# VincentStimper/normalizing-flows

Measured on NVIDIA H100. Metric: samples/sec forward_kld, 32-layer RQ-NSF d=64 batch=65536, higher is better.
Workload: dtype f32

## Files before the change

### normalizing-flows_b200/csrc/nfb_common.cuh

```cuda
#pragma once
#include <cuda_runtime.h>
#include <cuda_bf16.h>
#include <cuda_fp16.h>
#include <stdint.h>
#include <stdio.h>

#define NFB_OK 0
#define NFB_ERR_CUDA 1
#define NFB_ERR_ARG 2
#define NFB_ERR_UNSUPPORTED 3
#define NFB_ERR_STATE 4

void nfb_set_error(const char* fmt, ...);

#define NFB_CUDA(call)                                                                   \
    do {                                                                                 \
        cudaError_t e__ = (call);                                                        \
        if (e__ != cudaSuccess) {                                                        \
            nfb_set_error("%s:%d: %s -> %s", __FILE__, __LINE__, #call,                  \
                          cudaGetErrorString(e__));                                      \
            return NFB_ERR_CUDA;                                                         \
        }                                                                                \
    } while (0)

// ... 7 lines not shown

#define NFB_LAUNCH_CHECK() NFB_CUDA(cudaGetLastError())

namespace nfb {

constexpr float kMinBinWidth = 1e-3f;
constexpr float kMinBinHeight = 1e-3f;
constexpr float kMinDerivative = 1e-3f;
constexpr float kLog2e = 1.4426950408889634f;
constexpr float kLn2 = 0.6931471805599453f;

__device__ __forceinline__ uint32_t smem_u32(const void* p) {
    return static_cast<uint32_t>(__cvta_generic_to_shared(p));
}

__device__ __forceinline__ bool elect_one_sync() {
    uint32_t pred = 0;
    asm volatile(
        "{\n\t.reg .b32 %%rx;\n\t.reg .pred %%px;\n\t"
        "elect.sync %%rx|%%px, %1;\n\t"
        "@%%px mov.s32 %0, 1;\n\t}"
        : "+r"(pred)
        : "r"(0xffffffffu));
    return pred != 0;
}

__device__ __forceinline__ void mbar_init(uint32_t bar, uint32_t count) {
    asm volatile("mbarrier.init.shared::cta.b64 [%0], %1;" ::"r"(bar), "r"(count) : "memory");
}
__device__ __forceinline__ void fence_mbar_init() {
    asm volatile("fence.mbarrier_init.release.cluster;" ::: "memory");
}
__device__ __forceinline__ void mbar_arrive(uint32_t bar) {
    asm volatile("mbarrier.arrive.shared::cta.b64 _, [%0];" ::"r"(bar) : "memory");
}
__device__ __forceinline__ void mbar_expect_tx(uint32_t bar, uint32_t bytes) {
    asm volatile("mbarrier.arrive.expect_tx.shared::cta.b64 _, [%0], %1;" ::"r"(bar), "r"(bytes)
                 : "memory");
}
__device__ __forceinline__ bool mbar_try_wait(uint32_t bar, uint32_t parity) {
    uint32_t ok;
    asm volatile(
        "{\n\t.reg .pred p;\n\t"
        "mbarrier.try_wait.parity.shared::cta.b64 p, [%1], %2;\n\t"
        "selp.u32 %0, 1, 0, p;\n\t}"
        : "=r"(ok)
        : "r"(bar), "r"(parity)
        : "memory");
    return ok != 0;
}
static __device__ __noinline__ void fail_timeout(int* err, int tag) {
    if (err) atomicExch(err, tag);
    __threadfence_system();
    asm volatile("trap;");
}

__device__ __forceinline__ void mbar_wait(uint32_t bar, uint32_t parity, int* err, int tag) {
    if (mbar_try_wait(bar, parity)) return;
    long long t0 = clock64();
    while (!mbar_try_wait(bar, parity)) {
        if (clock64() - t0 > 4000000000LL) fail_timeout(err, tag);
    }
}

__device__ __forceinline__ void mbar_wait_warp(uint32_t bar, uint32_t parity, int* err, int tag) {
    if ((threadIdx.x & 31) == 0 && !mbar_try_wait(bar, parity)) {
        long long t0 = clock64();
        while (!mbar_try_wait(bar, parity)) {
            if (clock64() - t0 > 4000000000LL) fail_timeout(err, tag);
        }
    }
    __syncwarp();
}

__device__ __forceinline__ void bulk_g2s(uint32_t dst_smem, const void* src, uint32_t bytes,
                                         uint32_t bar) {
    asm volatile(
        "cp.async.bulk.shared::cluster.global.mbarrier::complete_tx::bytes [%0], [%1], %2, [%3];"
        ::"r"(dst_smem), "l"(src), "r"(bytes), "r"(bar)
        : "memory");
}
__device__ __forceinline__ void fence_proxy_async_smem() {
    asm volatile("fence.proxy.async.shared::cta;" ::: "memory");
}

__device__ __forceinline__ uint64_t wgmma_desc(uint32_t smem_addr, uint32_t lbo16 = 1, uint32_t sbo16 = 64) {
    return (uint64_t)((smem_addr & 0x3FFFFu) >> 4) | ((uint64_t)lbo16 << 16) | ((uint64_t)sbo16 << 32) | (1ull << 62);
}
__device__ __forceinline__ void wgmma_fence() { asm volatile("wgmma.fence.sync.aligned;" ::: "memory"); }
__device__ __forceinline__ void wgmma_commit() { asm volatile("wgmma.commit_group.sync.aligned;" ::: "memory"); }
template <int N> __device__ __forceinline__ void wgmma_wait() {
    asm volatile("wgmma.wait_group.sync.aligned %0;" ::"n"(N) : "memory");
}
template <int R> __device__ __forceinline__ void wgmma_hold(float (&d)[R]) {
#pragma unroll
    for (int i = 0; i < R; ++i) asm volatile("" : "+f"(d[i])::"memory");
}
__device__ __forceinline__ void wgmma_f16_n64(float (&d)[32], uint64_t a, uint64_t b, uint32_t scale_d) {
    asm volatile(
        "{\n\t.reg .pred p;\n\tsetp.ne.b32 p, %34, 0;\n\t"
        "wgmma.mma_async.sync.aligned.m64n64k16.f32.f16.f16 "
        "{"
        "%0,%1,%2,%3,%4,%5,%6,%7,%8,%9,%10,%11,%12,%13,%14,%15,"
        "%16,%17,%18,%19,%20,%21,%22,%23,%24,%25,%26,%27,%28,%29,%30,%31"
        "}, %32, %33, p, 1, 1, 0, 0;\n\t}"
        : "+f"(d[0]), "+f"(d[1]), "+f"(d[2]), "+f"(d[3]), "+f"(d[4]), "+f"(d[5]), "+f"(d[6]), "+f"(d[7]), "+f"(d[8]),
          "+f"(d[9]), "+f"(d[10]), "+f"(d[11]), "+f"(d[12]), "+f"(d[13]), "+f"(d[14]), "+f"(d[15]), "+f"(d[16]),
          "+f"(d[17]), "+f"(d[18]), "+f"(d[19]), "+f"(d[20]), "+f"(d[21]), "+f"(d[22]), "+f"(d[23]), "+f"(d[24]),
          "+f"(d[25]), "+f"(d[26]), "+f"(d[27]), "+f"(d[28]), "+f"(d[29]), "+f"(d[30]), "+f"(d[31])
        : "l"(a), "l"(b), "r"(scale_d));
}
__device__ __forceinline__ void wgmma_f16_n96(float (&d)[48], uint64_t a, uint64_t b, uint32_t scale_d) {
    asm volatile(
        "{\n\t.reg .pred p;\n\tsetp.ne.b32 p, %50, 0;\n\t"
        "wgmma.mma_async.sync.aligned.m64n96k16.f32.f16.f16 "
        "{"
        "%0,%1,%2,%3,%4,%5,%6,%7,%8,%9,%10,%11,%12,%13,%14,%15,"
        "%16,%17,%18,%19,%20,%21,%22,%23,%24,%25,%26,%27,%28,%29,%30,%31,"
        "%32,%33,%34,%35,%36,%37,%38,%39,%40,%41,%42,%43,%44,%45,%46,%47"
        "}, %48, %49, p, 1, 1, 0, 0;\n\t}"
        : "+f"(d[0]), "+f"(d[1]), "+f"(d[2]), "+f"(d[3]), "+f"(d[4]), "+f"(d[5]), "+f"(d[6]), "+f"(d[7]), "+f"(d[8]),
          "+f"(d[9]), "+f"(d[10]), "+f"(d[11]), "+f"(d[12]), "+f"(d[13]), "+f"(d[14]), "+f"(d[15]), "+f"(d[16]),
          "+f"(d[17]), "+f"(d[18]), "+f"(d[19]), "+f"(d[20]), "+f"(d[21]), "+f"(d[22]), "+f"(d[23]), "+f"(d[24]),
          "+f"(d[25]), "+f"(d[26]), "+f"(d[27]), "+f"(d[28]), "+f"(d[29]), "+f"(d[30]), "+f"(d[31]), "+f"(d[32]),
          "+f"(d[33]), "+f"(d[34]), "+f"(d[35]), "+f"(d[36]), "+f"(d[37]), "+f"(d[38]), "+f"(d[39]), "+f"(d[40]),
          "+f"(d[41]), "+f"(d[42]), "+f"(d[43]), "+f"(d[44]), "+f"(d[45]), "+f"(d[46]), "+f"(d[47])
        : "l"(a), "l"(b), "r"(scale_d));
}
__device__ __forceinline__ void wgmma_f16_n64_zero(float (&d)[32], uint64_t a, uint64_t b) {
    asm volatile(
        "wgmma.mma_async.sync.aligned.m64n64k16.f32.f16.f16 "
        "{"
        "%0,%1,%2,%3,%4,%5,%6,%7,%8,%9,%10,%11,%12,%13,%14,%15,"
        "%16,%17,%18,%19,%20,%21,%22,%23,%24,%25,%26,%27,%28,%29,%30,%31"
        "}, %32, %33, 0, 1, 1, 0, 0;"
        : "=f"(d[0]), "=f"(d[1]), "=f"(d[2]), "=f"(d[3]), "=f"(d[4]), "=f"(d[5]), "=f"(d[6]), "=f"(d[7]), "=f"(d[8]),
          "=f"(d[9]), "=f"(d[10]), "=f"(d[11]), "=f"(d[12]), "=f"(d[13]), "=f"(d[14]), "=f"(d[15]), "=f"(d[16]),
          "=f"(d[17]), "=f"(d[18]), "=f"(d[19]), "=f"(d[20]), "=f"(d[21]), "=f"(d[22]), "=f"(d[23]), "=f"(d[24]),
          "=f"(d[25]), "=f"(d[26]), "=f"(d[27]), "=f"(d[28]), "=f"(d[29]), "=f"(d[30]), "=f"(d[31])
        : "l"(a), "l"(b));
}
__device__ __forceinline__ void wgmma_f16_n96_zero(float (&d)[48], uint64_t a, uint64_t b) {
    asm volatile(
        "wgmma.mma_async.sync.aligned.m64n96k16.f32.f16.f16 "
        "{"
        "%0,%1,%2,%3,%4,%5,%6,%7,%8,%9,%10,%11,%12,%13,%14,%15,"
        "%16,%17,%18,%19,%20,%21,%22,%23,%24,%25,%26,%27,%28,%29,%30,%31,"
        "%32,%33,%34,%35,%36,%37,%38,%39,%40,%41,%42,%43,%44,%45,%46,%47"
        "}, %48, %49, 0, 1, 1, 0, 0;"
        : "=f"(d[0]), "=f"(d[1]), "=f"(d[2]), "=f"(d[3]), "=f"(d[4]), "=f"(d[5]), "=f"(d[6]), "=f"(d[7]), "=f"(d[8]),
          "=f"(d[9]), "=f"(d[10]), "=f"(d[11]), "=f"(d[12]), "=f"(d[13]), "=f"(d[14]), "=f"(d[15]), "=f"(d[16]),
          "=f"(d[17]), "=f"(d[18]), "=f"(d[19]), "=f"(d[20]), "=f"(d[21]), "=f"(d[22]), "=f"(d[23]), "=f"(d[24]),
          "=f"(d[25]), "=f"(d[26]), "=f"(d[27]), "=f"(d[28]), "=f"(d[29]), "=f"(d[30]), "=f"(d[31]), "=f"(d[32]),
          "=f"(d[33]), "=f"(d[34]), "=f"(d[35]), "=f"(d[36]), "=f"(d[37]), "=f"(d[38]), "=f"(d[39]), "=f"(d[40]),
          "=f"(d[41]), "=f"(d[42]), "=f"(d[43]), "=f"(d[44]), "=f"(d[45]), "=f"(d[46]), "=f"(d[47])
        : "l"(a), "l"(b));
}
template <int TA = 0, int TB = 0>
__device__ __forceinline__ void wgmma_bf16_n64(float (&d)[32], uint64_t a, uint64_t b, uint32_t scale_d, uint32_t on = 1) {
    asm volatile(
        "{\n\t.reg .pred p, q;\n\tsetp.ne.b32 p, %34, 0;\n\tsetp.ne.b32 q, %37, 0;\n\t"
        "@q wgmma.mma_async.sync.aligned.m64n64k16.f32.bf16.bf16 "
        "{"
        "%0,%1,%2,%3,%4,%5,%6,%7,%8,%9,%10,%11,%12,%13,%14,%15,"
        "%16,%17,%18,%19,%20,%21,%22,%23,%24,%25,%26,%27,%28,%29,%30,%31"
        "}, %32, %33, p, 1, 1, %35, %36;\n\t}"
// ... 61 lines not shown
```

### normalizing-flows_b200/csrc/nfb_fused_rqs.cu

```cuda
#include <type_traits>

#include "nfb_kernels.h"
#include "nfb_spline.cuh"

namespace nfb {

constexpr int kRows = kFusedTileRows;
constexpr int kCons = 256;
constexpr int kFusedThreads = kCons + 128;
constexpr int kProducerRegs = 24, kConsumerRegs = 240;
constexpr uint32_t kTileA = 8192;
constexpr uint32_t kSlotBytes = 32768;
constexpr uint32_t kSlots = 3;
constexpr uint32_t kOffW = 8 * kTileA;
constexpr uint32_t kOffX = kOffW + kSlots * kSlotBytes;
constexpr int kStgLd = 52;
constexpr uint32_t kStgBytes = kRows * kStgLd * 4;
constexpr uint32_t kOffStg = kOffX + kRows * 64 * 4;
constexpr uint32_t kOffMisc = kOffStg + 2 * kStgBytes;
constexpr uint32_t kOffBars = kOffMisc + 4 * kRows * 4;
constexpr uint32_t kNumBars = 10;
constexpr uint32_t kOffUnitQ = kOffBars + kNumBars * 8;
constexpr uint32_t kFusedSmem = kOffUnitQ + 32;
static_assert(kFusedSmem <= 232448, "shared memory budget");
static_assert(2 * kFusedFeaturesPerChunk * 24 * 64 * 4 <= (int)kSlotBytes, "final-layer record must fit a ring slot");

constexpr int kBarWFull = 0 , kBarWEmpty = 3 , kBarUnit = 6 ;

__device__ __forceinline__ uint32_t xs_index(int r, int c) { return r * 64 + (c ^ (r & 31)); }

__device__ __forceinline__ uint32_t a_chunk_off(int r, int c8) {
    return (r >> 3) * 1024 + (r & 7) * 128 + ((c8 ^ (r & 7)) << 4);
}

__device__ __forceinline__ void st_shared_v4(uint32_t addr, uint32_t a, uint32_t b, uint32_t c,
                                             uint32_t d) {
    asm volatile("st.shared.v4.b32 [%0], {%1,%2,%3,%4};" ::"r"(addr), "r"(a), "r"(b), "r"(c), "r"(d)
                 : "memory");
}
__device__ __forceinline__ void cons_bar_sync() {
    asm volatile("bar.sync 1, %0;" ::"n"(kCons) : "memory");
}
constexpr int kBarStgFull = 2, kBarStgFree = 3;
template <int ID> __device__ __forceinline__ void stg_bar_arrive() {
    __threadfence_block();
    asm volatile("bar.arrive %0, %1;" ::"n"(ID), "n"(kCons) : "memory");
}
template <int ID> __device__ __forceinline__ void stg_bar_wait() {
    asm volatile("bar.sync %0, %1;" ::"n"(ID), "n"(kCons) : "memory");
}
__device__ __forceinline__ void mbar_arrive_if(uint32_t bar, bool pred) {
    asm volatile("{\n\t.reg .pred p;\n\tsetp.ne.b32 p, %1, 0;\n\t@p mbarrier.arrive.shared::cta.b64 _, [%0];\n\t}"
                 ::"r"(bar), "r"((uint32_t)pred) : "memory");
}

__device__ __forceinline__ void split_store8(const float* v, uint32_t t0, uint32_t t1, uint32_t off) {
    uint32_t h[4], l[4];
#pragma unroll
    for (int i = 0; i < 4; ++i) {
        const float a = v[2 * i], b = v[2 * i + 1];
        h[i] = pack_f16x2(a, b);
        const float2 hf = unpack_f16x2(h[i]);
        l[i] = pack_f16x2(a - hf.x, b - hf.y);
    }
    st_shared_v4(t0 + off, h[0], h[1], h[2], h[3]);
    st_shared_v4(t1 + off, l[0], l[1], l[2], l[3]);
}
template <typename T> __device__ __forceinline__ T uniform(T v) {
    return (T)__shfl_sync(0xffffffffu, (int)v, 0);
}
__device__ __forceinline__ float pow2i(int e) { return __uint_as_float((uint32_t)(127 + e) << 23); }

struct MmaOps { uint32_t a_hi, a_lo, w_hi, w_lo, on, slabs; };
template <int SLABS, bool QUAD, int NREG, bool FIRST = false>
__device__ __forceinline__ void mma_record(float (&acc)[NREG], const MmaOps& x) {
    static_assert(NREG == 32 || NREG == 48, "N = 64 or 96");
    const uint64_t ah = wgmma_desc(x.a_hi), al = wgmma_desc(x.a_lo), bh = wgmma_desc(x.w_hi), bl = wgmma_desc(x.w_lo);
    auto pass = [&](uint64_t a, uint64_t b, bool opens) {
#pragma unroll
        for (int s = 0; s < SLABS; ++s) {
            if constexpr (NREG == 32) {
                if (FIRST && opens && s == 0) wgmma_f16_n64_zero(acc, a, b);
                else wgmma_f16_n64(acc, a + 2 * s, b + 2 * s, 1u);
            } else {
                if (FIRST && opens && s == 0) wgmma_f16_n96_zero(acc, a, b);
                else wgmma_f16_n96(acc, a + 2 * s, b + 2 * s, 1u);
            }
        }
    };
    pass(ah, bh, true);
    pass(al, bh, false);
    pass(ah, bl, false);
    if constexpr (QUAD) pass(al, bl, false);
}

enum { kClkClaim,
       kClkLoad,
       kClkLu,
       kClkHidRing,
       kClkHidMma,
       kClkHidEpi,
       kClkFinRing,
       kClkFinMma,
       kClkFinTail,
       kClkFinStage,
       kClkFinSpline,
       kClkStore,
       kClkProdEmpty,
       kClkProdOther,
       kClkUnits,
       kClkCount };
template <int RING, int MMA, int TAIL> struct WalkClk { static constexpr int ring = RING, mma = MMA, tail = TAIL; };
using LuClk = WalkClk<kClkLu, kClkLu, kClkLu>;
using HidClk = WalkClk<kClkHidRing, kClkHidMma, kClkHidMma>;
using FinClk = WalkClk<kClkFinRing, kClkFinMma, kClkFinTail>;
#ifdef NFB_PHASE_CLOCKS
__device__ unsigned long long g_phase_clocks[3][kClkCount];
struct PhaseClock {
    uint32_t last, sum[kClkCount];
    __device__ PhaseClock() {
        last = (uint32_t)clock64();
#pragma unroll
        for (int i = 0; i < kClkCount; ++i) sum[i] = 0;
    }
    template <int P> __device__ __forceinline__ void stamp() {
        const uint32_t t = (uint32_t)clock64();
        sum[P] += t - last;
        last = t;
    }
    __device__ void flush(int role) const {
#pragma unroll
        for (int i = 0; i < kClkCount; ++i) atomicAdd(&g_phase_clocks[role][i], (unsigned long long)sum[i]);
    }
};
#define NFB_CLK_BEGIN() PhaseClock clk
#define NFB_CLK(P) clk.template stamp<P>()
#define NFB_CLK_UNIT() (++clk.sum[kClkUnits])
#define NFB_CLK_END(role, pred) do { if (pred) clk.flush(role); } while (0)
#else
#define NFB_CLK_BEGIN() ((void)0)
#define NFB_CLK(P) ((void)0)
#define NFB_CLK_UNIT() ((void)0)
#define NFB_CLK_END(role, pred) ((void)0)
#endif

template <bool SAMPLE>
__global__ void __launch_bounds__(kFusedThreads, 1) fused_rqs_kernel(const FusedParams p) {
    extern __shared__ __align__(1024) uint8_t smem[];
    const uint32_t sbase = smem_u32(smem);
    const int warp = uniform((int)(threadIdx.x >> 5)), lane = threadIdx.x & 31;
    float* xs = reinterpret_cast<float*>(smem + kOffX);
    float* ldsum = reinterpret_cast<float*>(smem + kOffMisc);
    int* rowexp = reinterpret_cast<int*>(smem + kOffMisc + 3 * kRows * 4);
    float* rowmax = reinterpret_cast<float*>(smem + kOffStg);
    const uint32_t bars = sbase + kOffBars;
    auto bar = [bars](int i) { return bars + 8u * i; };

    if ((sbase & 1023u) != 0) {
        if (threadIdx.x == 0 && p.err) atomicExch(p.err, 900);
        return;
    }
    if (threadIdx.x == 0) {
        for (int i = 0; i < (int)kSlots; ++i) {
            mbar_init(bar(kBarWFull + i), 1);
            mbar_init(bar(kBarWEmpty + i), 2);
        }
        for (int i = 0; i < 4; ++i) mbar_init(bar(kBarUnit + i), 1);
        fence_mbar_init();
    }
    __syncthreads();

    volatile int* unit_q = reinterpret_cast<volatile int*>(smem + kOffUnitQ);
    if (warp >= kCons / 32) {
        setmaxnreg_dec<kProducerRegs>();
        if (warp != kCons / 32) return;
        const long long n_tiles = (p.rows + kRows - 1) / kRows;
        const long long n_units = n_tiles * p.n_layers;
        auto decode = [&](long long u, int& cursor, int& layer, long long& tile) {
            if (!p.wave_order) {
                layer = (int)(u / n_tiles);
                tile = u - (long long)layer * n_tiles;
                return;
            }
            while (cursor + 1 < p.wave_elems && u >= (long long)__ldg(p.wave_order + 2 * (cursor + 1) + 1)) ++cursor;
            const uint32_t w = __ldg(p.wave_order + 2 * cursor);
            layer = (int)(w & 0xffu);
            tile = (long long)(w >> 8) * p.wave_tpg + (u - (long long)__ldg(p.wave_order + 2 * cursor + 1));
        };
        uint32_t slot = 0, par = 0;
        int wcur = 0;
        NFB_CLK_BEGIN();
        for (uint32_t ui = 0;; ++ui) {
            long long u;
            if (p.ticket) {
                int t = 0;
                if (lane == 0) t = atomicAdd(p.ticket, 1);
                u = (long long)__shfl_sync(0xffffffffu, t, 0);
            } else {
                u = (long long)blockIdx.x + (long long)ui * gridDim.x;
            }
            const bool more = u < n_units;
            int ulayer = -1;
            long long utile = 0;
            if (more) decode(u, wcur, ulayer, utile);
            if (lane == 0) {
                unit_q[2 * (ui & 3u)] = ulayer;
                unit_q[2 * (ui & 3u) + 1] = (int)utile;
                mbar_arrive(bar(kBarUnit + (ui & 3u)));
            }
            __syncwarp();
            if (!more) break;
            NFB_CLK_UNIT();
            const FusedLayer& L = p.layers[ulayer];
            const FusedStep* steps = L.steps;
            const int n_steps = L.n_steps;
            const int lu_steps = L.has_lu ? 1 : 0;
            const int reps = (SAMPLE && L.ar_passes > 0) ? L.ar_passes : 1;
            const int total = n_steps ? lu_steps + reps * (n_steps - lu_steps) : 0;
            const uint32_t lu_bytes = L.has_lu ? 2u * 8192u : 0u;
            int s = 0;
            uint32_t off = 0;
            uint32_t bytes = total ? (uint32_t)__ldg(&steps[0].bytes16) << 4 : 0u;
            for (int i = 0; i < total; ++i) {
                int sn = s + 1;
                uint32_t offn = off + bytes;
                if (sn == n_steps) { sn = lu_steps; offn = lu_bytes; }
                const uint32_t nbytes = i + 1 < total ? (uint32_t)__ldg(&steps[sn].bytes16) << 4 : 0u;
                NFB_CLK(kClkProdOther);
                mbar_wait(bar(kBarWEmpty + slot), par ^ 1, p.err, 100 + slot);
                NFB_CLK(kClkProdEmpty);
                if (elect_one_sync()) {
                    mbar_expect_tx(bar(kBarWFull + slot), bytes);
                    bulk_g2s(sbase + kOffW + slot * kSlotBytes, L.wstream + off, bytes, bar(kBarWFull + slot));
                }
                __syncwarp();
                s = sn;
                off = offn;
                bytes = nbytes;
                if (++slot == kSlots) { slot = 0; par ^= 1; }
            }
        }
        NFB_CLK(kClkProdOther);
        NFB_CLK_END(2, lane == 0);
        return;
    }

    setmaxnreg_inc<kConsumerRegs>();
    const int et = threadIdx.x;
    const int wg = uniform(et >> 7);
    const int wl = warp & 3;
    const int ra = 16 * wl + (lane >> 2);
    const int rb = ra + 8;
    const int cq = 2 * (lane & 3);
    const uint32_t aA = sbase;
    float* stg0 = reinterpret_cast<float*>(smem + kOffStg);
    uint32_t slot = 0, wpar = 0;
    NFB_CLK_BEGIN();

    for (uint32_t ui = 0;; ++ui) {
        mbar_wait(bar(kBarUnit + (ui & 3u)), (ui >> 2) & 1u, p.err, 600 + (int)(ui & 3u));
        const int layer = uniform(unit_q[2 * (ui & 3u)]);
        const long long tile = uniform(unit_q[2 * (ui & 3u) + 1]);
        if (layer < 0) break;
        NFB_CLK_UNIT();
        const FusedLayer& L = p.layers[layer];
        const int D = L.D;
        auto own = [&](int q) { return uniform((int)L.own[wg][q]); };
        const int n_steps = uniform(L.n_steps), lu_steps = uniform(L.has_lu ? 1 : 0);
        const int n_hidden = uniform(L.n_hidden), n_pairs = uniform(L.n_chunks >> 1);
        int sidx = 0;
        auto hand_back = [&](auto arrivals, int s, bool pred) {
#pragma unroll
            for (int i = 0; i < decltype(arrivals)::value; ++i) mbar_arrive_if(bar(kBarWEmpty + s), pred && (et & 127) == 0);
        };
        auto walk_records = [&](auto issue, auto arrivals, auto phases, int& prev, auto open, auto retire) {
            using Clk = decltype(phases);
            auto record = [&](auto first) {
                union { uint2 raw; FusedStep s; } st;
                st.raw = __ldg(reinterpret_cast<const uint2*>(L.steps) + sidx);
                st.raw.x = uniform(st.raw.x);
                st.raw.y = uniform(st.raw.y);
                sidx = sidx + 1 == n_steps ? lu_steps : sidx + 1;
                NFB_CLK(Clk::mma);
                mbar_wait(bar(kBarWFull + slot), wpar, p.err, 220 + slot);
                NFB_CLK(Clk::ring);
                wgmma_fence();
                const bool last = issue(st.s, first);
                if constexpr (decltype(first)::value) NFB_CLK(Clk::mma);
                wgmma_wait<1>();
                hand_back(arrivals, prev < 0 ? 0 : prev, prev >= 0);
                if constexpr (decltype(first)::value) NFB_CLK(Clk::tail);
                prev = (int)slot;
                if (++slot == kSlots) { slot = 0; wpar ^= 1; }
                return last;
            };
            bool last = false;
            if constexpr (decltype(open)::value) {
                last = record(std::true_type());
                retire();
            }
            while (!last) last = record(std::false_type());
        };
        auto half_ops = [&](const FusedStep& s, int h) {
            const uint32_t kc = h ? s.kc1 : s.kc, fl = h ? s.flags1 : s.flags;
            const uint32_t w = sbase + kOffW + slot * kSlotBytes + ((fl & kStepHalf) ? 0u : (uint32_t)h * s.n8 * 1024u);
            return MmaOps{aA + kc * kTileA, aA + (4 + kc) * kTileA, w, w + ((uint32_t)s.bytes16 << 3),
                          (uint32_t)!(fl & kStepSkip), 4u - ((fl >> kStepSlabShift) & 3u)};
        };
        auto slice_products = [&](float (&acc)[32], auto opens, auto quad) {
            return [&](const FusedStep& s, auto first) {
                constexpr bool Q = decltype(quad)::value;
                const MmaOps x = half_ops(s, wg);
                if constexpr (decltype(first)::value && decltype(opens)::value) {
                    mma_record<4, Q, 32, true>(acc, x);
                    wgmma_commit();
                } else if (x.on) {
                    mma_record<4, Q, 32>(acc, x);
                    wgmma_commit();
                } else {
                    wgmma_commit();
                }
                return ((wg ? s.flags1 : s.flags) & kStepLast) != 0;
            };
        };
        auto no_products = [&](const FusedStep& s, auto) {
            wgmma_commit();
            return ((wg ? s.flags1 : s.flags) & kStepLast) != 0;
        };
        using One = std::integral_constant<int, 1>;
        using NoQuad = std::integral_constant<bool, false>;

        float* zdst = p.zout + (long long)layer * p.z_stride;
        const float* zsrc = layer == 0 ? p.zin : p.zout + (long long)(layer - 1) * p.z_stride;
        const long long row0 = tile * kRows;
        const int r = et & (kRows - 1);
        const int rq = et >> 6;
        const long long grow = row0 + r;
        const bool row_live = grow < p.rows;

        if (layer > 0) {
            if (lane == 0) {
                const int* flag = p.progress + tile;
                int seen;
                const long long t0 = clock64();
                do {
                    asm volatile("ld.acquire.gpu.global.s32 %0, [%1];" : "=r"(seen) : "l"(flag) : "memory");
                    if (seen < layer && clock64() - t0 > 4000000000LL) fail_timeout(p.err, 500);
                } while (seen < layer);
            }
            __syncwarp();
            {
                int seen;
                asm volatile("ld.acquire.gpu.global.s32 %0, [%1];" : "=r"(seen) : "l"(p.progress + tile) : "memory");
                if (seen < layer) fail_timeout(p.err, 501);
            }
        }
        if (layer == 0 && p.in_ready) {
            const int need = (int)min(row0 + kRows, p.rows);
            if (lane == 0) {
                int seen;
                const long long t0 = clock64();
                do {
                    asm volatile("ld.acquire.sys.global.s32 %0, [%1];" : "=r"(seen) : "l"(p.in_ready) : "memory");
                    if (seen < need && clock64() - t0 > 20000000000LL) fail_timeout(p.err, 510);
                } while (seen < need);
            }
            __syncwarp();
            {
                int seen;
                asm volatile("ld.acquire.sys.global.s32 %0, [%1];" : "=r"(seen) : "l"(p.in_ready) : "memory");
                if (seen < need) fail_timeout(p.err, 511);
            }
        }
        NFB_CLK(kClkClaim);
        float lq_old = 0.f;
        if (rq == 2 && row_live && (layer > 0 || p.accumulate)) lq_old = __ldcg(p.logq + grow);
        if (D == 64) {
            float4 v[kRows * 16 / kCons];
#pragma unroll
            for (int k = 0; k < kRows * 16 / kCons; ++k) {
                const int i4 = et + k * kCons, rr = i4 >> 4;
                const long long gr = row0 + rr;
                v[k] = gr < p.rows ? __ldcg(reinterpret_cast<const float4*>(zsrc + gr * 64) + (i4 & 15))
                                   : make_float4(0.f, 0.f, 0.f, 0.f);
            }
#pragma unroll
            for (int k = 0; k < kRows * 16 / kCons; ++k) {
                const int i4 = et + k * kCons, rr = i4 >> 4, c0 = (i4 & 15) * 4;
                xs[xs_index(rr, c0)] = v[k].x;
                xs[xs_index(rr, c0 + 1)] = v[k].y;
                xs[xs_index(rr, c0 + 2)] = v[k].z;
                xs[xs_index(rr, c0 + 3)] = v[k].w;
                float m = fmaxf(fmaxf(fabsf(v[k].x), fabsf(v[k].y)), fmaxf(fabsf(v[k].z), fabsf(v[k].w)));
                m = fmaxf(m, __shfl_xor_sync(0xffffffffu, m, 1));
                m = fmaxf(m, __shfl_xor_sync(0xffffffffu, m, 2));
                m = fmaxf(m, __shfl_xor_sync(0xffffffffu, m, 4));
                m = fmaxf(m, __shfl_xor_sync(0xffffffffu, m, 8));
                if ((et & 15) == 0) rowmax[rr] = m;
            }
        } else {
            for (int i = et; i < kRows * D; i += kCons) {
                const int rr = i / D, cc = i - rr * D;
                const long long gr = row0 + rr;
                xs[xs_index(rr, cc)] = gr < p.rows ? __ldcg(zsrc + gr * D + cc) : 0.f;
            }
        }
        cons_bar_sync();
        auto set_row_exp = [&](float zmax) {
            int e = (int)((__float_as_uint(zmax) >> 23) & 0xffu) - 126;
            rowexp[r] = max(0, min(126, e));
        };
        if (rq == 0) {
            float zmax = 0.f;
            if (D == 64) zmax = rowmax[r];
            else
                for (int c = 0; c < D; ++c) zmax = fmaxf(zmax, fabsf(xs[xs_index(r, c)]));
            set_row_exp(zmax);
        }
        cons_bar_sync();
        auto ru = [&](float s, int row) { return s * pow2i(-rowexp[row]); };
        auto ruinv = [&](float s, int row) { return s * pow2i(rowexp[row]); };
        auto get_x = [&](int c) -> float { return xs[xs_index(r, c)]; };
        auto put_y = [&](int c, float y) { xs[xs_index(r, c)] = y; };
        const int ar = et >> 2, aq = et & 3;
        auto store_a = [&](auto value, float sc_base) {
            const float sc = ru(sc_base, ar);
            float v[16];
#pragma unroll
            for (int j = 0; j < 16; ++j) v[j] = value(aq * 16 + j) * sc;
#pragma unroll
            for (int g = 0; g < 2; ++g) split_store8(v + 8 * g, aA, aA + 4 * kTileA, a_chunk_off(ar, 2 * aq + g));
            fence_proxy_async_smem();
            cons_bar_sync();
        };
        auto build_a_net = [&]() {
            store_a([&](int k) {
                const int c = L.in_idx[k];
                return c >= 0 ? xs[xs_index(ar, c)] : 0.f;
            }, L.a_sc[1]);
        };
        float ladsum = 0.f, lad_even = 0.f;
        const bool folded = uniform(!SAMPLE && L.has_lu && L.fold_lu);
        if (lu_steps) {
            store_a([&](int k) { return k < D ? xs[xs_index(ar, k)] : 0.f; }, L.a_sc[0]);
            NFB_CLK(kClkLoad);
            int prev = -1;
            if (wg == 0) {
                float acc[32];
                walk_records(slice_products(acc, std::true_type(), std::true_type()), One(), LuClk(), prev,
                             std::true_type(), [] {});
                wgmma_wait<0>();
                hand_back(One(), prev, true);
                wgmma_hold(acc);
                const float ia = ruinv(L.a_inv[0], ra), ib = ruinv(L.a_inv[0], rb);
#pragma unroll
                for (int i = 0; i < 32; ++i) {
                    const int c = 8 * (i >> 2) + cq + (i & 1);
                    const int rr = (i & 2) ? rb : ra;
                    if (c < D) xs[xs_index(rr, c)] = fmaf(acc[i], (i & 2) ? ib : ia, __ldg(L.bias_lu + c));
                }
            } else {
                walk_records(no_products, One(), LuClk(), prev, std::false_type(), [] {});
                wgmma_wait<0>();
                hand_back(One(), prev, true);
            }
            cons_bar_sync();
            NFB_CLK(kClkLu);
        }
// ... 169 lines not shown
                int prev = -1;
                auto pair = [&](float (&acc)[48], float (&done)[48], int ci) __attribute__((always_inline)) {
                    walk_records(products(acc), Two(), FinClk(), prev, std::true_type(), [&] { stage(done, ci - 1); });
                };
                auto finish = [&](float (&acc)[48], int ci) {
                    wgmma_wait<0>();
                    hand_back(Two(), prev, true);
                    NFB_CLK(kClkFinTail);
                    stage(acc, ci);
                };
                float accA[48], accB[48];
                if (n_pairs > 0) {
                    load_bias(0);
                    walk_records(products(accA), Two(), FinClk(), prev, std::true_type(), [] {});
                    for (int ci = 1;; ci += 2) {
                        if (ci == n_pairs) { finish(accA, ci - 1); break; }
                        pair(accB, accA, ci);
                        if (ci + 1 == n_pairs) { finish(accB, ci); break; }
                        pair(accA, accB, ci + 1);
                    }
                }
            } else {
                if (n_pairs > 0) {
                    const uint32_t adv = slot + (uint32_t)(n_steps - sidx);
                    slot = adv % kSlots;
                    wpar ^= (adv / kSlots) & 1u;
                    sidx = lu_steps;
                }
                const int f = (et >> 6) & 1;
                lad_even = ldsum[f * kRows + r];
                const int F = L.F, T = L.T;
                for (int ci = 0; ci < n_pairs; ++ci) {
                    stg_bar_wait<kBarStgFull>();
                    float pv[2][24];
#pragma unroll
                    for (int h = 0; h < 2; ++h) {
                        const float4* sp = reinterpret_cast<const float4*>(stg0 + (h * kRows + r) * kStgLd + 24 * f);
#pragma unroll
                        for (int q = 0; q < 6; ++q) {
                            const float4 s4 = sp[q];
                            pv[h][4 * q] = s4.x;
                            pv[h][4 * q + 1] = s4.y;
                            pv[h][4 * q + 2] = s4.z;
                            pv[h][4 * q + 3] = s4.w;
                        }
                    }
                    if (ci + 1 < n_pairs) stg_bar_arrive<kBarStgFree>();
                    NFB_CLK(kClkFinStage);
                    const int t0 = 2 * ci * F + f;
                    auto splines = [&](auto lanes) {
                        constexpr int N = decltype(lanes)::value;
                        int col[N];
                        float xin[N], y[N], l[N];
#pragma unroll
                        for (int h = 0; h < N; ++h) {
                            col[h] = L.tr_idx[t0 + h * F];
                            xin[h] = get_x(col[h]);
                            if (arsamp) xin[h] = row_live ? __ldcg(zdst + grow * D + col[h]) : 0.f;
                        }
                        rqs_core_lanes<N, 8, SAMPLE>(xin, [&pv](int h, int i) { return pv[h][i]; },
                                                     [&pv](int h, int i) { return pv[h][8 + i]; },
                                                     [&pv](int h, int i) { return pv[h][16 + i]; }, L.tail, y, l);
#pragma unroll
                        for (int h = 0; h < N; ++h) put_y(col[h], y[h]);
                        lad_even += l[0];
                        if constexpr (N == 2) ladsum += l[1];
                    };
                    if (t0 + F < T) splines(std::integral_constant<int, 2>());
                    else if (t0 < T) splines(std::integral_constant<int, 1>());
                    NFB_CLK(kClkFinSpline);
                }
            }
            cons_bar_sync();
        }
        NFB_CLK(kClkFinStage);
        if (rq == 3) {
            ldsum[r] = lad_even;
            ldsum[kRows + r] = ladsum;
        }
        cons_bar_sync();
        if (rq == 2 && row_live) {
            const float tot = lad_even + ldsum[r] + ladsum + ldsum[kRows + r] +
                              (L.lu_logdet ? __ldg(L.lu_logdet) : 0.f);
            __stcg(p.logq + grow, tot + lq_old);
        }
        store_tile();
        if (p.progress) __threadfence();
        cons_bar_sync();
        if (p.progress && et == 0) {
            __threadfence();
            asm volatile("st.release.gpu.global.s32 [%0], %1;" ::"l"(p.progress + tile), "r"(layer + 1) : "memory");
        }
        NFB_CLK(kClkStore);
    }
    NFB_CLK_END(wg, (et & 127) == 0);
}

int launch_fused_rqs(const FusedParams& p, int sm_count, int sample, cudaStream_t st) {
    static PerDevice per_dev;
    const int dev_sms = per_dev.ensure([] {
        cudaError_t e = cudaFuncSetAttribute(fused_rqs_kernel<false>, cudaFuncAttributeMaxDynamicSharedMemorySize,
                                             (int)kFusedSmem);
        if (e == cudaSuccess)
            e = cudaFuncSetAttribute(fused_rqs_kernel<true>, cudaFuncAttributeMaxDynamicSharedMemorySize, (int)kFusedSmem);
        return e;
    });
    if (dev_sms < 0) return NFB_ERR_CUDA;
    if (sm_count <= 0 || sm_count > dev_sms) sm_count = dev_sms;
    NFB_CHECK(p.n_layers >= 1 && (p.n_layers == 1 || p.progress), NFB_ERR_ARG, "fused rqs: bad layer list");
    const long long n_tiles = (p.rows + kRows - 1) / kRows;
    if (n_tiles == 0) return NFB_OK;
    const long long n_units = n_tiles * p.n_layers;
    const unsigned grid = (unsigned)(n_units < sm_count ? n_units : sm_count);
    if (sample) fused_rqs_kernel<true><<<grid, kFusedThreads, kFusedSmem, st>>>(p);
    else fused_rqs_kernel<false><<<grid, kFusedThreads, kFusedSmem, st>>>(p);
    NFB_LAUNCH_CHECK();
    return NFB_OK;
}

#ifdef NFB_PHASE_CLOCKS
extern "C" __attribute__((visibility("default"))) int nfb_phase_clocks_read(unsigned long long* out, int reset) {
    NFB_CUDA(cudaDeviceSynchronize());
    if (out) NFB_CUDA(cudaMemcpyFromSymbol(out, g_phase_clocks, sizeof(g_phase_clocks)));
    if (reset) {
        const unsigned long long zero[3][kClkCount] = {};
        NFB_CUDA(cudaMemcpyToSymbol(g_phase_clocks, zero, sizeof(zero)));
    }
    return NFB_OK;
}
extern "C" __attribute__((visibility("default"))) int nfb_phase_clocks_count() { return kClkCount; }
#endif

__global__ void build_effective_kernel(const float* __restrict__ W, const float* __restrict__ M,
                                       int src_cols, const int* __restrict__ src_row,
                                       const int* __restrict__ src_col,
                                       const float* __restrict__ row_scale, float* __restrict__ E,
                                       int n_pad, int k_pad, float gain) {
    const int idx = blockIdx.x * blockDim.x + threadIdx.x;
    if (idx >= n_pad * k_pad) return;
    const int i = idx / k_pad, j = idx - i * k_pad;
    const int sr = src_row[i], sc = src_col[j];
    float v = 0.f;
    if (sr >= 0 && sc >= 0) {
        const long long o = (long long)sr * src_cols + sc;
        v = W[o];
        if (M) v *= M[o];
        if (row_scale) v *= row_scale[i];
        v *= gain;
    }
    E[idx] = v;
}
__global__ void swizzle_split_kernel(const float* __restrict__ E, int n_pad, int k_pad,
                                     int rows_per_rec, int nsplit, float scale, uint8_t* __restrict__ out) {
    const int kcs = k_pad / 64;
    const long long total = (long long)n_pad * k_pad;
    const long long idx = (long long)blockIdx.x * blockDim.x + threadIdx.x;
    if (idx >= total) return;
    const int i = (int)(idx / k_pad), j = (int)(idx - (long long)i * k_pad);
    const int rb = i / rows_per_rec, rr = i - rb * rows_per_rec;
    const int kc = j >> 6, kk = j & 63;
    const float v = E[idx] * scale;
    const size_t rec_bytes = (size_t)rows_per_rec * 128;
    const size_t in_rec = (size_t)(rr >> 3) * 1024 + (rr & 7) * 128 + (((kk >> 3) ^ (rr & 7)) << 4) +
                          (kk & 7) * 2;
    float rem = v;
    for (int s = 0; s < nsplit; ++s) {
        const __half h = __float2half_rn(rem);
        rem -= __half2float(h);
        const size_t rec = ((size_t)rb * kcs + kc) * nsplit + s;
        *reinterpret_cast<__half*>(out + rec * rec_bytes + in_rec) = h;
    }
}

__global__ void pack_records_kernel(const float* __restrict__ E, int k_pad, const PackRec* __restrict__ recs, float scale,
                                    uint8_t* __restrict__ base) {
// ... 95 lines not shown
```

Baseline: 5.497 million.

## Double-buffer tile I/O with bulk async loader and publisher warps

Adds two producer-side warps. One prefetches the next unit's z tile and logq slice into a second shared-memory buffer with cp.async.bulk, after first waiting on the layer-progress flag. The other writes the finished tile and logq back to global memory with bulk stores and then publishes progress, so consumers no longer do per-thread global loads, stores and threadfences. The intent is to overlap global I/O with the spline/GEMM compute of the adjacent unit. The cost is double the tile and logq buffers, extra mbarriers, an un-swizzle pass through shared memory before store, and more complex cross-warp synchronisation.

```diff
diff --git a/normalizing-flows_b200/csrc/nfb_common.cuh b/normalizing-flows_b200/csrc/nfb_common.cuh
--- a/normalizing-flows_b200/csrc/nfb_common.cuh
+++ b/normalizing-flows_b200/csrc/nfb_common.cuh
@@ -113,6 +113,18 @@
 }
 __device__ __forceinline__ void fence_proxy_async_smem() {
     asm volatile("fence.proxy.async.shared::cta;" ::: "memory");
+}
+__device__ __forceinline__ void fence_proxy_async_global() {
+    asm volatile("fence.proxy.async.global;" ::: "memory");
+}
+__device__ __forceinline__ void bulk_s2g(void* dst, uint32_t src_smem, uint32_t bytes) {
+    asm volatile("cp.async.bulk.global.shared::cta.bulk_group [%0], [%1], %2;" ::"l"(dst), "r"(src_smem), "r"(bytes)
+                 : "memory");
+}
+__device__ __forceinline__ void bulk_commit() { asm volatile("cp.async.bulk.commit_group;" ::: "memory"); }
+template <bool READ> __device__ __forceinline__ void bulk_wait_all() {
+    if constexpr (READ) asm volatile("cp.async.bulk.wait_group.read 0;" ::: "memory");
+    else asm volatile("cp.async.bulk.wait_group 0;" ::: "memory");
 }
 
 __device__ __forceinline__ uint64_t wgmma_desc(uint32_t smem_addr, uint32_t lbo16 = 1, uint32_t sbo16 = 64) {
diff --git a/normalizing-flows_b200/csrc/nfb_fused_rqs.cu b/normalizing-flows_b200/csrc/nfb_fused_rqs.cu
--- a/normalizing-flows_b200/csrc/nfb_fused_rqs.cu
+++ b/normalizing-flows_b200/csrc/nfb_fused_rqs.cu
@@ -13,19 +13,23 @@
 constexpr uint32_t kSlotBytes = 32768;
 constexpr uint32_t kSlots = 3;
 constexpr uint32_t kOffW = 8 * kTileA;
+constexpr uint32_t kTileBytes = kRows * 64 * 4;
 constexpr uint32_t kOffX = kOffW + kSlots * kSlotBytes;
 constexpr int kStgLd = 52;
 constexpr uint32_t kStgBytes = kRows * kStgLd * 4;
-constexpr uint32_t kOffStg = kOffX + kRows * 64 * 4;
+constexpr uint32_t kOffStg = kOffX + 2 * kTileBytes;
 constexpr uint32_t kOffMisc = kOffStg + 2 * kStgBytes;
-constexpr uint32_t kOffBars = kOffMisc + 4 * kRows * 4;
-constexpr uint32_t kNumBars = 10;
+constexpr uint32_t kOffLq = kOffMisc + 4 * kRows * 4;
+constexpr uint32_t kOffBars = kOffLq + 2 * kRows * 4;
+constexpr uint32_t kNumBars = 16;
 constexpr uint32_t kOffUnitQ = kOffBars + kNumBars * 8;
-constexpr uint32_t kFusedSmem = kOffUnitQ + 32;
+constexpr uint32_t kOffPubQ = kOffUnitQ + 32;
+constexpr uint32_t kFusedSmem = kOffPubQ + 16;
 static_assert(kFusedSmem <= 232448, "shared memory budget");
 static_assert(2 * kFusedFeaturesPerChunk * 24 * 64 * 4 <= (int)kSlotBytes, "final-layer record must fit a ring slot");
 
 constexpr int kBarWFull = 0 , kBarWEmpty = 3 , kBarUnit = 6 ;
+constexpr int kBarTileFull = 10 , kBarOutFull = 12 , kBarTileFree = 14 ;
 
 __device__ __forceinline__ uint32_t xs_index(int r, int c) { return r * 64 + (c ^ (r & 31)); }
 
@@ -144,12 +148,30 @@
 #define NFB_CLK_END(role, pred) ((void)0)
 #endif
 
+struct UnitIo {
+    const float* src;
+    float* dst;
+    long long row0;
+    int rows;
+    bool bulk;
+};
+__device__ __forceinline__ UnitIo unit_io(const FusedParams& p, int layer, long long tile, int D, bool arsamp) {
+    UnitIo u;
+    u.dst = p.zout + (long long)layer * p.z_stride;
+    u.src = layer == 0 ? p.zin : p.zout + (long long)(layer - 1) * p.z_stride;
+    u.row0 = tile * kRows;
+    u.rows = (int)min((long long)kRows, p.rows - u.row0);
+    const uintptr_t a = (uintptr_t)(u.src + u.row0 * D) | (uintptr_t)(u.dst + u.row0 * D) | (uintptr_t)(p.logq + u.row0);
+    u.bulk = D == 64 && !arsamp && (u.rows & 3) == 0 && (a & 15u) == 0;
+    return u;
+}
+
 template <bool SAMPLE>
 __global__ void __launch_bounds__(kFusedThreads, 1) fused_rqs_kernel(const FusedParams p) {
     extern __shared__ __align__(1024) uint8_t smem[];
     const uint32_t sbase = smem_u32(smem);
     const int warp = uniform((int)(threadIdx.x >> 5)), lane = threadIdx.x & 31;
-    float* xs = reinterpret_cast<float*>(smem + kOffX);
+    float* const xs0 = reinterpret_cast<float*>(smem + kOffX);
     float* ldsum = reinterpret_cast<float*>(smem + kOffMisc);
     int* rowexp = reinterpret_cast<int*>(smem + kOffMisc + 3 * kRows * 4);
     float* rowmax = reinterpret_cast<float*>(smem + kOffStg);
@@ -166,13 +188,91 @@
             mbar_init(bar(kBarWEmpty + i), 2);
         }
         for (int i = 0; i < 4; ++i) mbar_init(bar(kBarUnit + i), 1);
+        for (int i = 0; i < 2; ++i) {
+            mbar_init(bar(kBarTileFull + i), 1);
+            mbar_init(bar(kBarOutFull + i), 1);
+            mbar_init(bar(kBarTileFree + i), 1);
+        }
         fence_mbar_init();
     }
     __syncthreads();
 
     volatile int* unit_q = reinterpret_cast<volatile int*>(smem + kOffUnitQ);
+    volatile int* pub_q = reinterpret_cast<volatile int*>(smem + kOffPubQ);
+    float* const lqs0 = reinterpret_cast<float*>(smem + kOffLq);
     if (warp >= kCons / 32) {
         setmaxnreg_dec<kProducerRegs>();
+        if (warp == kCons / 32 + 1) {
+            for (uint32_t ui = 0;; ++ui) {
+                const uint32_t b = ui & 1u;
+                mbar_wait_warp(bar(kBarUnit + (ui & 3u)), (ui >> 2) & 1u, p.err, 610 + (int)(ui & 3u));
+                const int layer = unit_q[2 * (ui & 3u)];
+                const long long tile = unit_q[2 * (ui & 3u) + 1];
+                mbar_wait_warp(bar(kBarTileFree + b), ((ui >> 1) & 1u) ^ 1u, p.err, 620 + (int)b);
+                bool bulk = false;
+                UnitIo io{};
+                int D = 0;
+                if (layer >= 0) {
+                    const FusedLayer& L = p.layers[layer];
+                    D = L.D;
+                    io = unit_io(p, layer, tile, D, SAMPLE && L.ar_passes > 0);
+                    bulk = io.bulk;
+                }
+                if (bulk && lane == 0) {
+                    const long long t0 = clock64();
+                    int seen;
+                    if (layer > 0) {
+                        do {
+                            asm volatile("ld.acquire.gpu.global.s32 %0, [%1];" : "=r"(seen) : "l"(p.progress + tile) : "memory");
+                            if (seen < layer && clock64() - t0 > 4000000000LL) fail_timeout(p.err, 502);
+                        } while (seen < layer);
+                    } else if (p.in_ready) {
+                        const int need = (int)(io.row0 + io.rows);
+                        do {
+                            asm volatile("ld.acquire.sys.global.s32 %0, [%1];" : "=r"(seen) : "l"(p.in_ready) : "memory");
+                            if (seen < need && clock64() - t0 > 20000000000LL) fail_timeout(p.err, 512);
+                        } while (seen < need);
+                    }
+                    fence_proxy_async_global();
+                    const uint32_t zb = (uint32_t)io.rows * D * 4u, lb = (uint32_t)io.rows * 4u;
+                    mbar_expect_tx(bar(kBarTileFull + b), zb + lb);
+                    bulk_g2s(sbase + kOffX + b * kTileBytes, io.src + io.row0 * D, zb, bar(kBarTileFull + b));
+                    bulk_g2s(sbase + kOffLq + b * kRows * 4u, p.logq + io.row0, lb, bar(kBarTileFull + b));
+                } else if (lane == 0) {
+                    mbar_arrive(bar(kBarTileFull + b));
+                }
+                __syncwarp();
+                if (layer < 0) return;
+            }
+        }
+        if (warp == kCons / 32 + 2) {
+            for (uint32_t ui = 0;; ++ui) {
+                const uint32_t b = ui & 1u;
+                mbar_wait_warp(bar(kBarOutFull + b), (ui >> 1) & 1u, p.err, 630 + (int)b);
+                const int layer = pub_q[2 * b];
+                const long long tile = pub_q[2 * b + 1];
+                if (layer < 0) return;
+                const FusedLayer& L = p.layers[layer];
+                const int D = L.D;
+                const UnitIo io = unit_io(p, layer, tile, D, SAMPLE && L.ar_passes > 0);
+                if (lane == 0) {
+                    if (io.bulk) {
+                        bulk_s2g(io.dst + io.row0 * D, sbase + kOffX + b * kTileBytes, (uint32_t)io.rows * D * 4u);
+                        bulk_s2g(p.logq + io.row0, sbase + kOffLq + b * kRows * 4u, (uint32_t)io.rows * 4u);
+                        bulk_commit();
+                        bulk_wait_all<true>();
+                        mbar_arrive(bar(kBarTileFree + b));
+                        bulk_wait_all<false>();
+                        fence_proxy_async_global();
+                        if (p.progress)
+                            asm volatile("st.release.gpu.global.s32 [%0], %1;" ::"l"(p.progress + tile), "r"(layer + 1) : "memory");
+                    } else {
+                        mbar_arrive(bar(kBarTileFree + b));
+                    }
+                }
+                __syncwarp();
+            }
+        }
         if (warp != kCons / 32) return;
         const long long n_tiles = (p.rows + kRows - 1) / kRows;
         const long long n_units = n_tiles * p.n_layers;
@@ -261,8 +361,22 @@
         mbar_wait(bar(kBarUnit + (ui & 3u)), (ui >> 2) & 1u, p.err, 600 + (int)(ui & 3u));
         const int layer = uniform(unit_q[2 * (ui & 3u)]);
         const long long tile = uniform(unit_q[2 * (ui & 3u) + 1]);
-        if (layer < 0) break;
+        const uint32_t tb = ui & 1u;
+        mbar_wait(bar(kBarTileFull + tb), (ui >> 1) & 1u, p.err, 640 + (int)tb);
+        auto to_publisher = [&]() {
+            if (et == 0) {
+                pub_q[2 * tb] = layer;
+                pub_q[2 * tb + 1] = (int)tile;
+                mbar_arrive(bar(kBarOutFull + tb));
+            }
+        };
+        if (layer < 0) {
+            to_publisher();
+            break;
+        }
         NFB_CLK_UNIT();
+        float* const xs = xs0 + tb * (kTileBytes / 4);
+        float* const lqs = lqs0 + tb * kRows;
         const FusedLayer& L = p.layers[layer];
         const int D = L.D;
         auto own = [&](int q) { return uniform((int)L.own[wg][q]); };
@@ -337,8 +451,9 @@
         const int rq = et >> 6;
         const long long grow = row0 + r;
         const bool row_live = grow < p.rows;
-
-        if (layer > 0) {
+        const bool bulk = uniform((int)unit_io(p, layer, tile, D, SAMPLE && L.ar_passes > 0).bulk);
+
+        if (!bulk && layer > 0) {
             if (lane == 0) {
                 const int* flag = p.progress + tile;
                 int seen;
@@ -355,7 +470,7 @@
                 if (seen < layer) fail_timeout(p.err, 501);
             }
         }
-        if (layer == 0 && p.in_ready) {
+        if (!bulk && layer == 0 && p.in_ready) {
             const int need = (int)min(row0 + kRows, p.rows);
             if (lane == 0) {
                 int seen;
@@ -374,16 +489,18 @@
         }
         NFB_CLK(kClkClaim);
         float lq_old = 0.f;
-        if (rq == 2 && row_live && (layer > 0 || p.accumulate)) lq_old = __ldcg(p.logq + grow);
+        if (rq == 2 && row_live && (layer > 0 || p.accumulate)) lq_old = bulk ? lqs[r] : __ldcg(p.logq + grow);
         if (D == 64) {
             float4 v[kRows * 16 / kCons];
 #pragma unroll
             for (int k = 0; k < kRows * 16 / kCons; ++k) {
                 const int i4 = et + k * kCons, rr = i4 >> 4;
                 const long long gr = row0 + rr;
-                v[k] = gr < p.rows ? __ldcg(reinterpret_cast<const float4*>(zsrc + gr * 64) + (i4 & 15))
-                                   : make_float4(0.f, 0.f, 0.f, 0.f);
-            }
+                v[k] = gr >= p.rows ? make_float4(0.f, 0.f, 0.f, 0.f)
+                       : bulk      ? reinterpret_cast<const float4*>(xs)[i4]
+                                   : __ldcg(reinterpret_cast<const float4*>(zsrc + gr * 64) + (i4 & 15));
+            }
+            if (bulk) cons_bar_sync();
 #pragma unroll
             for (int k = 0; k < kRows * 16 / kCons; ++k) {
                 const int i4 = et + k * kCons, rr = i4 >> 4, c0 = (i4 & 15) * 4;
@@ -719,15 +836,31 @@
         if (rq == 2 && row_live) {
             const float tot = lad_even + ldsum[r] + ladsum + ldsum[kRows + r] +
                               (L.lu_logdet ? __ldg(L.lu_logdet) : 0.f);
-            __stcg(p.logq + grow, tot + lq_old);
-        }
-        store_tile();
-        if (p.progress) __threadfence();
+            if (bulk) lqs[r] = tot + lq_old;
+            else __stcg(p.logq + grow, tot + lq_old);
+        }
+        if (bulk) {
+            float4 v[kRows * 16 / kCons];
+#pragma unroll
+            for (int k = 0; k < kRows * 16 / kCons; ++k) {
+                const int i4 = et + k * kCons, rr = i4 >> 4, c0 = (i4 & 15) * 4;
+                v[k] = make_float4(xs[xs_index(rr, c0)], xs[xs_index(rr, c0 + 1)], xs[xs_index(rr, c0 + 2)],
+                                   xs[xs_index(rr, c0 + 3)]);
+            }
+            cons_bar_sync();
+#pragma unroll
+            for (int k = 0; k < kRows * 16 / kCons; ++k) reinterpret_cast<float4*>(xs)[et + k * kCons] = v[k];
+        } else {
+            store_tile();
+            if (p.progress) __threadfence();
+        }
+        fence_proxy_async_smem();
         cons_bar_sync();
-        if (p.progress && et == 0) {
+        if (!bulk && p.progress && et == 0) {
             __threadfence();
             asm volatile("st.release.gpu.global.s32 [%0], %1;" ::"l"(p.progress + tile), "r"(layer + 1) : "memory");
         }
+        to_publisher();
         NFB_CLK(kClkStore);
     }
     NFB_CLK_END(wg, (et & 127) == 0);
```

Result: no change. 5.524 million, median of 6 (+0.5%).
